# xiaochuanle/MECAT

Measured on AMD Instinct MI355X. Metric: candidate overlaps/sec, higher is better.
Workload: dtype int32

## Files before the change

### mecat_amd/csrc/seed_strand.hip

```cpp
#include <stdlib.h>

#include <algorithm>

#include "seed_defs.h"
#include "seed_replay.h"
#include "seed_walk.h"

#define FS_CAP 8192
#define FS_SEGCAP 6144
#define FS_SMALLN 16
#define FS_BIGN 512
#define FS_BIGCAP 768
#define FS_GATECAP 1024
#define FS_OVF16 0x8000u
#ifndef FS_Q1
#define FS_LPB1 8
#define FS_NP1 4
#define FS_Q1 2
#define FS_D1 2
#define FS_LPB2 8
#define FS_NP2 4
#define FS_Q2 2
#define FS_D2 2
#endif

struct FsLds {
    union {
        uint32_t cnt32[FLT_M / 2];
        struct {
            uint32_t pay[FS_CAP];
            uint16_t eslot[FS_CAP];
            uint16_t big[FS_BIGCAP];
            uint32_t hist[FS_WAVES][64];
            uint64_t tf[FS_GATECAP];
        } e;
    } x;
    union {
        uint32_t cur32[FS_CAP / 2];
        uint16_t perm[FS_SEGCAP];
    } y;
    uint32_t occ[REL_WORDS];
    uint32_t rel[REL_WORDS];
    uint16_t base_ci[REL_WORDS];
    uint32_t sq_id[FS_SEGCAP];
    uint16_t sq_st[FS_SEGCAP + 2];
    uint16_t sq_score[FS_SEGCAP];
    uint16_t gate[FS_GATECAP];
    uint32_t qpos[FS_WAVES][128];
    uint16_t qkm[FS_WAVES][128];
    uint32_t wtot[FS_WAVES];
    unsigned long long red[FS_WAVES];
    unsigned long long tally[3];
    uint32_t misc[12];
};
static_assert(sizeof(FsLds) <= 160 * 1024 - 512, "one workgroup per CU");

struct FusedCtl { unsigned long long alloc; unsigned int n_fallback; unsigned int next ; unsigned long long prof[32]; };
#ifdef FS_PROF
#define FS_MARK(i) do { __syncthreads(); if (threadIdx.x == 0) { const unsigned long long t_ = wall_clock64(); atomicAdd(&ctl->prof[(i) + 16 * (s & 1)], t_ - t_prev); t_prev = t_; } } while (0)
#else
#define FS_MARK(i) do { } while (0)
#endif

__device__ __forceinline__ void fs_block_sum2(const int tid, uint32_t a, uint32_t b, unsigned long long* red , uint32_t* sa, uint32_t* sb) {
    const int lane = tid & 63;
    for (int o = 32; o > 0; o >>= 1) {
        a += (uint32_t)__builtin_amdgcn_ds_bpermute((lane ^ o) << 2, (int)a);
        b += (uint32_t)__builtin_amdgcn_ds_bpermute((lane ^ o) << 2, (int)b);
    }
    const unsigned long long v = (unsigned long long)a | ((unsigned long long)b << 32);
    if (lane == 0) red[tid >> 6] = v;
    __syncthreads();
    unsigned long long t = 0;
#pragma unroll
    for (int w = 0; w < FS_WAVES; ++w) t += red[w];
    *sa = (uint32_t)t;
    *sb = (uint32_t)(t >> 32);
}

struct FsStrand { int rid, off, len, K, cut_byte; bool rev; };
__device__ __forceinline__ FsStrand fs_strand(const mhip_offset_t* __restrict__ roffs, const ReadSel& sel, int ib, int s, bool cuts, int cut_step) {
    FsStrand d;
    d.rid = sel_rid(sel, ib + (s >> 1));
    d.off = roffs[d.rid].offset;
    d.len = roffs[d.rid].size;
    d.K = kmers_of(d.len);
    d.rev = s & 1;
    d.cut_byte = 7;
    if (cuts) {
        const long long need = (long long)d.off + d.len + 1 + 5 * ZV;
        const long long t = (need + cut_step - 1) / cut_step;
        if (t <= 7) d.cut_byte = (int)t - 1;
    }
    return d;
}
__device__ __forceinline__ int64_t fs_kmer_at(const FsStrand& d, int km) {
    return !d.rev ? (int64_t)d.off + (int64_t)km * BC : (int64_t)d.off + d.len - MHIP_KMER_SIZE - (int64_t)km * BC;
}
__device__ __forceinline__ void fs_hdr_words(const uint32_t* __restrict__ pac, const FsStrand& d, int km, uint32_t (&w)[2]) {
    const int64_t i = fs_kmer_at(d, km) >> 4;
    w[0] = pac[i];
    w[1] = pac[i + 1];
}
__device__ __forceinline__ void fs_hdr_record(const uint32_t* __restrict__ starts, const uint4* __restrict__ recs, const FsStrand& d, int km,
                                              const uint32_t (&w)[2], uint32_t (&r)[3]) {
    const uint64_t W = ((uint64_t)__builtin_bswap32(w[0]) << 32) | __builtin_bswap32(w[1]);
    uint32_t id = (uint32_t)(W >> (64 - 26 - (int)((fs_kmer_at(d, km) & 15) << 1))) & KMER_MASK;
    if (d.rev) id = kmer_revcomp(id);
    if (recs) {
        const uint4 v = recs[id];
        r[0] = v.x; r[1] = v.y; r[2] = v.z;
    } else {
        r[0] = starts[id]; r[1] = starts[id + 1];
    }
}
__device__ __forceinline__ void fs_hdr_decode(bool cuts, const FsStrand& d, const uint32_t (&r)[3], uint32_t* bs, uint32_t* cnt, uint32_t* all) {
    *bs = r[0];
    if (cuts) {
        *all = r[2] >> 24;
        *cnt = ((d.cut_byte < 4 ? r[1] : r[2]) >> (8 * (d.cut_byte & 3))) & 0xFFu;
    } else {
        *all = *cnt = r[1] - r[0];
    }
}

template <int NQ>
__device__ __forceinline__ void fs_bitonic(uint32_t* p, const uint32_t n, const int lane) {
    uint32_t v[NQ];
#pragma unroll
    for (int q = 0; q < NQ; ++q) { const uint32_t idx = q * 64 + lane; v[q] = idx < n ? p[idx] : 0xFFFFFFFFu; }
#pragma unroll
    for (int k = 2; k <= NQ * 64; k <<= 1) {
#pragma unroll
        for (int j = k >> 1; j > 0; j >>= 1) {
            if (j >= 64) {
                const int dq = j >> 6;
#pragma unroll
                for (int q = 0; q < NQ; ++q) {
                    if ((q & dq) == 0) {
                        const uint32_t a = v[q], b = v[q | dq];
                        const bool asc = ((q * 64) & k) == 0;
                        v[q] = asc ? min(a, b) : max(a, b);
                        v[q | dq] = asc ? max(a, b) : min(a, b);
                    }
                }
            } else {
#pragma unroll
                for (int q = 0; q < NQ; ++q) {
                    const uint32_t o = (uint32_t)__builtin_amdgcn_ds_bpermute((lane ^ j) << 2, (int)v[q]);
                    const bool asc = (((q * 64 + lane) & k) == 0), lower = (lane & j) == 0;
                    v[q] = (asc == lower) ? min(v[q], o) : max(v[q], o);
                }
            }
        }
    }
    __builtin_amdgcn_wave_barrier();
#pragma unroll
    for (int q = 0; q < NQ; ++q) { const uint32_t idx = q * 64 + lane; if (idx < n) p[idx] = v[q]; }
}

__device__ __forceinline__ uint32_t fs_cnt(const uint32_t* cnt32, uint32_t e) { return (cnt32[e >> 1] >> ((e & 1u) * 16u)) & 0xFFFFu; }

#define FS_UNI(x) ((uint32_t)__builtin_amdgcn_readfirstlane((int)(x)))
__global__ __launch_bounds__(FS_THREADS) void seed_strand(const uint32_t* __restrict__ pac, const mhip_offset_t* __restrict__ roffs, ReadSel sel,
                                                          int ib, int ns, const uint32_t* __restrict__ starts, const uint4* __restrict__ recs,
                                                          int cut_step, const uint16_t* __restrict__ slots, const int32_t* __restrict__ offsets,
                                                          SeedArrays A, int gate, int hi_bits, int min_kmer_match, double cutoff,
                                                          unsigned long long cap, FusedCtl* __restrict__ ctl,
                                                          unsigned long long* __restrict__ counters, RefReads R) {
    __shared__ FsLds L;
    const int tid0 = threadIdx.x;
    const bool probed = A.km_bstart != nullptr;
    const bool cuts = recs != nullptr;
    uint32_t* const hbs = L.sq_id;
    uint16_t* const hcn = L.sq_score;
    constexpr int PF = 2;
    uint32_t pw[PF][2], pr[PF][3];
#pragma unroll
    for (int j = 0; j < PF; ++j) { pw[j][0] = pw[j][1] = 0; pr[j][0] = pr[j][1] = pr[j][2] = 0; }
    int pf = -1;
    if (tid0 == 0) { L.tally[0] = L.tally[1] = L.tally[2] = 0; L.misc[8] = atomicAdd(&ctl->next, 1u); L.misc[9] = atomicAdd(&ctl->next, 1u); }
    __syncthreads();
    int s = (int)min(FS_UNI(L.misc[8]), (uint32_t)ns), sn = (int)min(FS_UNI(L.misc[9]), (uint32_t)ns), s2 = ns;
    for (; s < ns; s = sn, sn = s2) {
    __syncthreads();
    int tid = tid0;
    asm volatile("" : "+v"(tid));
    const int lane = tid & 63, wv = __builtin_amdgcn_readfirstlane(tid >> 6);
    const FsStrand d = fs_strand(roffs, sel, ib, s, cuts, cut_step);
    const int rid = d.rid, rlen = d.len, K = d.K;
    auto fail = [&]() {
        if (tid == 0) { A.fused[s] = 0; atomicAdd(&ctl->n_fallback, 1u); atomicAdd(&counters[14], 1ull); }
    };
    unsigned long long t_prev = wall_clock64(); (void)t_prev;
    for (int i = tid; i < FLT_M / 2; i += FS_THREADS) L.x.cnt32[i] = 0;
    for (int i = tid; i < REL_WORDS; i += FS_THREADS) L.rel[i] = 0u;
    if (tid < 8) L.misc[tid] = 0;
    if (tid == 0) L.misc[8] = atomicAdd(&ctl->next, 1u);
    uint32_t Hall, run_all;
    {
        const bool room = K <= FS_SEGCAP;
        uint32_t hc = 0, ha = 0;
        if (probed) {
            const uint32_t kb = A.km_base[s];
            for (int km = tid; km < K; km += FS_THREADS) {
                const uint32_t bs = A.km_bstart[kb + km], cn = A.km_cnt[kb + km];
                hc += cn;
                if (room) { hbs[km] = bs; hcn[km] = (uint16_t)cn; }
            }
        } else {
            auto take = [&](int km, const uint32_t (&r)[3]) {
                uint32_t bs, cn, al;
                fs_hdr_decode(cuts, d, r, &bs, &cn, &al);
                hc += cn;
                ha += al;
                if (room) { hbs[km] = bs; hcn[km] = (uint16_t)cn; }
            };
            if (pf != s) {
#pragma unroll
                for (int j = 0; j < PF; ++j)
                    if (tid + j * FS_THREADS < K) fs_hdr_words(pac, d, tid + j * FS_THREADS, pw[j]);
#pragma unroll
                for (int j = 0; j < PF; ++j)
                    if (tid + j * FS_THREADS < K) fs_hdr_record(starts, recs, d, tid + j * FS_THREADS, pw[j], pr[j]);
            }
#pragma unroll
            for (int j = 0; j < PF; ++j) asm volatile("" : "+v"(pr[j][0]), "+v"(pr[j][1]), "+v"(pr[j][2]));
#pragma unroll
            for (int j = 0; j < PF; ++j)
                if (tid + j * FS_THREADS < K) take(tid + j * FS_THREADS, pr[j]);
            for (int km = tid + PF * FS_THREADS; km < K; km += FS_THREADS) {
                uint32_t w[2], r[3] = {0, 0, 0};
                fs_hdr_words(pac, d, km, w);
                fs_hdr_record(starts, recs, d, km, w, r);
                take(km, r);
            }
        }
        fs_block_sum2(tid, hc, ha, L.red, &Hall, &run_all);
        Hall = FS_UNI(Hall);
        run_all = FS_UNI(run_all);
        s2 = (int)min(FS_UNI(L.misc[8]), (uint32_t)ns);
        if (!probed && tid == 0) { L.tally[0] += (unsigned long long)K; L.tally[1] += run_all; L.tally[2] += Hall; A.strand_hits_all[s] = Hall; }
    }
    if (Hall == 0) {
        if (tid == 0) { A.fused[s] = 1; A.strand_hits[s] = 0; A.hit_base[s] = 0; A.nseg[s] = 0; A.nrec[s] = 0; A.ngated[s] = 0; }
        continue;
    }
    if (Hall >= 65536u || K > 32767 || K > FS_SEGCAP) { fail(); continue; }

    FS_MARK(0);
    fs_walk<FS_LPB1, FS_NP1, FS_Q1, FS_D1, false>(tid, hbs, hcn, slots, K, [&](int, uint32_t e) { atomicAdd(&L.x.cnt32[e >> 1], 1u << ((e & 1u) * 16u)); });
    __syncthreads();
    FS_MARK(1);

    static_assert(FLT_M / FS_THREADS == 32, "one bitmap word per thread");
    uint32_t cw[18];
    {
        const uint4* c4 = (const uint4*)&L.x.cnt32[16 * tid];
#pragma unroll
        for (int q = 0; q < 4; ++q) { const uint4 v = c4[q]; cw[1 + 4 * q] = v.x; cw[2 + 4 * q] = v.y; cw[3 + 4 * q] = v.z; cw[4 + 4 * q] = v.w; }
        cw[0] = L.x.cnt32[(16 * tid - 1) & (FLT_M / 2 - 1)];
        cw[17] = L.x.cnt32[(16 * tid + 16) & (FLT_M / 2 - 1)];
        uint32_t hot = 0;
        {
#pragma unroll
        for (int j = 1; j <= 16; ++j) {
            const int lo = (int)(cw[j] & 0xFFFFu), hi = (int)(cw[j] >> 16), pl = (int)(cw[j - 1] >> 16), nx = (int)(cw[j + 1] & 0xFFFFu);
            const bool hl = lo > 0 && (lo + hi >= gate || lo + pl >= gate);
            const bool hh = hi > 0 && (hi + nx >= gate || hi + lo >= gate);
            hot |= (hl ? 1u : 0u) << (2 * (j - 1)) | (hh ? 1u : 0u) << (2 * (j - 1) + 1);
        }
        const uint32_t reach = (uint32_t)min(sweep_reach(rlen), FLT_M / 2 - 1);
        for (uint32_t m = hot; m; m &= m - 1u) {
            const uint32_t e = (uint32_t)tid * 32u + (uint32_t)__builtin_ctz(m);
            uint32_t lo = (e - reach) & (FLT_M - 1), left = 2 * reach + 1;
            while (left > 0) {
                const uint32_t b = lo & 31u, take = min(32u - b, left);
                const uint32_t msk = (take == 32u ? 0xFFFFFFFFu : ((1u << take) - 1u)) << b;
                atomicOr(&L.rel[lo >> 5], msk);
                lo = (lo + take) & (FLT_M - 1);
                left -= take;
            }
        }
        }
    }
    __syncthreads();
    FS_MARK(2);
    uint32_t kept;
    {
        const uint32_t r = L.rel[tid];
        uint32_t occ = 0, mine = 0;
        bool toolong = false;
#pragma unroll
        for (int j = 0; j < 32; ++j) {
            const uint32_t h = (cw[1 + (j >> 1)] >> ((j & 1) * 16)) & 0xFFFFu;
            if (((r >> j) & 1u) && h) { occ |= 1u << j; mine += h; toolong |= h > FS_BIGN; }
        }
        uint32_t both;
        const uint32_t exb = fs_excl_scan(tid, mine | ((uint32_t)__popc(occ) << 16), L.wtot, &both);
        const uint32_t ex = exb & 0xFFFFu, cx = exb >> 16;
        kept = FS_UNI(both) & 0xFFFFu;
        if (kept > FS_CAP) { fail(); continue; }
        L.occ[tid] = occ;
        L.base_ci[tid] = (uint16_t)cx;
        uint16_t* cur16 = (uint16_t*)L.y.cur32;
        uint32_t at = ex, ci = cx;
        if (occ) {
#pragma unroll
            for (int j = 0; j < 32; ++j) {
                const uint32_t h = (cw[1 + (j >> 1)] >> ((j & 1) * 16)) & 0xFFFFu;
                if ((occ >> j) & 1u) { cur16[ci++] = (uint16_t)at; at += h; }
            }
        }
        if (toolong) L.misc[3] = 1;
        __syncthreads();
        if (FS_UNI(L.misc[3])) { fail(); continue; }
    }
    if (kept == 0) {
        if (tid == 0) { A.fused[s] = 1; A.strand_hits[s] = 0; A.hit_base[s] = 0; A.nseg[s] = 0; A.nrec[s] = 0; A.ngated[s] = 0; }
        continue;
    }
    if (tid == 0) {
        const unsigned long long hb0 = atomicAdd(&ctl->alloc, (unsigned long long)kept);
        if (hb0 + kept > cap) L.misc[3] = 1;
        L.misc[6] = (uint32_t)hb0;
        L.misc[7] = (uint32_t)(hb0 >> 32);
    }
    __syncthreads();
    if (FS_UNI(L.misc[3])) { fail(); continue; }
    const uint64_t hb = ((uint64_t)L.misc[7] << 32) | L.misc[6];

    FS_MARK(3);
    const bool ahead = !probed && sn < ns;
    FsStrand dn = d;
    if (ahead) {
        dn = fs_strand(roffs, sel, ib, sn, cuts, cut_step);
#pragma unroll
        for (int j = 0; j < PF; ++j)
            if (tid + j * FS_THREADS < dn.K) fs_hdr_words(pac, dn, tid + j * FS_THREADS, pw[j]);
    }
    {
        uint32_t qn = 0;
        auto place = [&](uint32_t qi) {
            const uint32_t pos = L.qpos[wv][qi], km = L.qkm[wv][qi];
            const uint32_t seg = pos / (uint32_t)ZV, off = pos - seg * (uint32_t)ZV;
            const uint32_t e = seg & (FLT_M - 1), w = e >> 5, b = e & 31u;
            const uint32_t oc = L.occ[w];
            const uint32_t ci = (uint32_t)L.base_ci[w] + (uint32_t)__popc(oc & ((1u << b) - 1u));
            const uint32_t sh = (ci & 1u) * 16u;
            const uint32_t p = (atomicAdd(&L.y.cur32[ci >> 1], 1u << sh) >> sh) & 0xFFFFu;
            L.x.e.pay[p] = ((seg >> FLT_BITS) << 26) | (km << 11) | off;
            L.x.e.eslot[p] = (uint16_t)e;
        };
        fs_walk<FS_LPB2, FS_NP2, FS_Q2, FS_D2, true>(tid, hbs, hcn, offsets, K, [&](int km, uint32_t pos, bool valid) {
            const uint32_t seg = pos / (uint32_t)ZV;
            const uint32_t e = seg & (FLT_M - 1);
            const uint32_t oc = valid ? L.occ[e >> 5] : 0u;
            const bool keep = (bool)((oc >> (e & 31u)) & 1u);
            const unsigned long long m = __builtin_amdgcn_ballot_w64(keep);
            if (m) {
                if (keep) {
                    const uint32_t at = qn + (uint32_t)__popcll(m & ((1ull << lane) - 1ull));
                    L.qpos[wv][at] = pos;
                    L.qkm[wv][at] = (uint16_t)km;
                }
                qn += (uint32_t)__popcll(m);
                if (qn >= 64u) { qn -= 64u; place(qn + (uint32_t)lane); }
            }
        });
        if ((uint32_t)lane < qn) place((uint32_t)lane);
    }
    if (ahead) {
#pragma unroll
        for (int j = 0; j < PF; ++j)
            if (tid + j * FS_THREADS < dn.K) fs_hdr_record(starts, recs, dn, tid + j * FS_THREADS, pw[j], pr[j]);
        pf = sn;
    }
    __syncthreads();
    FS_MARK(4);
    {
        const uint16_t* cur16 = (const uint16_t*)L.y.cur32;
        uint32_t val[FS_CAP / FS_THREADS], dst[FS_CAP / FS_THREADS];
#pragma unroll
        for (int rd = 0; rd < FS_CAP / FS_THREADS; ++rd) {
            const uint32_t i = (uint32_t)rd * FS_THREADS + tid;
            dst[rd] = 0xFFFFFFFFu;
            val[rd] = 0;
            if ((uint32_t)rd * FS_THREADS < kept && i < kept) {
                const uint32_t v = L.x.e.pay[i], e = L.x.e.eslot[i], w = e >> 5, oc = L.occ[w];
                const uint32_t ci = (uint32_t)L.base_ci[w] + (uint32_t)__popc(oc & ((1u << (e & 31u)) - 1u));
                const uint32_t st = ci ? cur16[ci - 1] : 0u, en = cur16[ci], n = en - st;
                if (n > FS_SMALLN) {
                    if (i == st) L.x.e.big[atomicAdd(&L.misc[0], 1u)] = (uint16_t)ci;
                } else if (n > 1) {
                    uint32_t rank = 0;
                    for (uint32_t k = st; k < en; ++k) rank += L.x.e.pay[k] < v ? 1u : 0u;
                    val[rd] = v;
                    dst[rd] = st + rank;
                }
            }
        }
        __syncthreads();
#pragma unroll
        for (int rd = 0; rd < FS_CAP / FS_THREADS; ++rd)
            if (dst[rd] != 0xFFFFFFFFu) L.x.e.pay[dst[rd]] = val[rd];
        FS_MARK(11);
        const uint32_t nbig = L.misc[0];
        for (uint32_t k = wv; k < nbig; k += FS_WAVES) {
            const uint32_t ci = L.x.e.big[k];
            const uint32_t st = ci ? cur16[ci - 1] : 0u, n = (uint32_t)cur16[ci] - st;
            if (n <= 64) fs_bitonic<1>(L.x.e.pay + st, n, lane);
            else if (n <= 256) fs_bitonic<4>(L.x.e.pay + st, n, lane);
            else fs_bitonic<8>(L.x.e.pay + st, n, lane);
        }
        __syncthreads();
    }

    FS_MARK(5);
    uint32_t nrec, nseg;
    {
        constexpr int CHMAX = FS_CAP / FS_THREADS;
        const uint32_t ch = (kept + FS_THREADS - 1) / FS_THREADS;
        const uint32_t i0 = (uint32_t)tid * ch;
        uint32_t pv[CHMAX], sv[CHMAX];
        uint32_t ppay = 0, psl = 0xFFFFFFFFu;
        if (i0 > 0 && i0 < kept) { ppay = L.x.e.pay[i0 - 1]; psl = L.x.e.eslot[i0 - 1]; }
        uint32_t hm = 0, rm = 0;
#pragma unroll
        for (int c = 0; c < CHMAX; ++c) {
            const uint32_t i = i0 + c;
            const bool in = (uint32_t)c < ch && i < kept;
            pv[c] = in ? L.x.e.pay[i] : 0u;
            sv[c] = in ? L.x.e.eslot[i] : 0u;
            const bool head = in && (sv[c] != psl || (pv[c] >> 26) != (ppay >> 26));
            const bool rec = in && (head || ((pv[c] >> 11) & 0x7FFFu) != ((ppay >> 11) & 0x7FFFu));
            hm |= (head ? 1u : 0u) << c;
            rm |= (rec ? 1u : 0u) << c;
            if (in) { ppay = pv[c]; psl = sv[c]; }
        }
        uint32_t both;
        const uint32_t ex = fs_excl_scan(tid, (uint32_t)__popc(rm) | ((uint32_t)__popc(hm) << 16), L.wtot, &both);
        uint32_t rpos = ex & 0xFFFFu, spos = ex >> 16;
        both = FS_UNI(both);
        nrec = both & 0xFFFFu;
        nseg = both >> 16;
        if (nseg > FS_SEGCAP) { fail(); continue; }
#pragma unroll
        for (int c = 0; c < CHMAX; ++c) {
            if ((rm >> c) & 1u) {
                if ((hm >> c) & 1u) {
                    L.sq_id[spos] = ((pv[c] >> 26) << FLT_BITS) | sv[c];
                    L.sq_st[spos] = (uint16_t)rpos;
                    ++spos;
                }
                L.x.e.pay[rpos++] = ((pv[c] & 0x7FFu) << 16) | ((((pv[c] >> 11) & 0x7FFFu) + 1u) & 0xFFFFu);
            }
        }
        if (tid == 0) L.sq_st[nseg] = (uint16_t)nrec;
    }
    uint16_t* perm = L.y.perm;
    __syncthreads();

    FS_MARK(6);
    if (hi_bits == 0) {
        for (uint32_t q = tid; q < nseg; q += FS_THREADS) perm[q] = (uint16_t)q;
    } else {
        uint32_t* hist = &L.x.e.hist[0][0];
        hist[tid] = 0;
        __syncthreads();
        const uint32_t chunk = (((nseg + FS_WAVES - 1) / FS_WAVES) + 63u) & ~63u;
        const uint32_t lo = min(nseg, (uint32_t)wv * chunk), hi = min(nseg, lo + chunk);
        for (uint32_t q = lo + lane; q < hi; q += 64) atomicAdd(&L.x.e.hist[wv][L.sq_id[q] >> FLT_BITS], 1u);
        __syncthreads();
        {
            const uint32_t bin = tid >> 4, w = tid & 15;
            static_assert(FS_WAVES == 16, "16 waves");
            const uint32_t v = L.x.e.hist[w][bin];
            uint32_t all;
            const uint32_t ex = fs_excl_scan(tid, v, L.wtot, &all);
            L.x.e.hist[w][bin] = ex;
        }
        __syncthreads();
        volatile uint32_t* cur = L.x.e.hist[wv];
        const uint64_t lt = (1ull << lane) - 1ull;
        for (uint32_t q0 = lo; q0 < hi; q0 += 64) {
            const uint32_t q = q0 + lane;
            const bool valid = q < hi;
            const uint32_t d = valid ? L.sq_id[q] >> FLT_BITS : 0u;
            uint64_t peers = __ballot(valid);
            for (int b = 0; b < hi_bits; ++b) {
                const uint64_t m = __ballot((d >> b) & 1u);
                peers &= ((d >> b) & 1u) ? m : ~m;
            }
            const uint32_t rank = __popcll(peers & lt);
            const uint32_t base = valid ? cur[d] : 0u;
            if (valid) perm[base + rank] = (uint16_t)q;
            if (valid && rank == 0) cur[d] = base + (uint32_t)__popcll(peers);
        }
    }
    FS_MARK(7);
    uint16_t* ovf = L.x.e.big;
    for (uint32_t q = tid; q < nseg; q += FS_THREADS) {
        const uint32_t c = (uint32_t)L.sq_st[q + 1] - (uint32_t)L.sq_st[q];
        if (c > SM) {
            const uint32_t k = atomicAdd(&L.misc[1], 1u);
            if (k < FS_BIGCAP) ovf[k] = (uint16_t)q;
            L.sq_score[q] = (uint16_t)FS_OVF16;
        } else {
            L.sq_score[q] = (uint16_t)c;
        }
    }
    __syncthreads();
    if (FS_UNI(L.misc[1]) > FS_BIGCAP) { fail(); continue; }
    {
        const uint32_t novf = L.misc[1];
        for (uint32_t k = wv; k < novf; k += FS_WAVES) {
            const uint32_t q = ovf[k];
            const uint32_t st = L.sq_st[q], en = L.sq_st[q + 1];
            int sc;
            replay_overflow(L.x.e.pay + st, (int)(en - st), A.ent_fin + hb + st, A.escore + hb + st, cutoff, &sc);
            if (lane == 0) L.sq_score[q] = (uint16_t)((uint32_t)sc | FS_OVF16);
        }
    }
    __syncthreads();
    FS_MARK(8);
    for (uint32_t g = tid; g < nseg; g += FS_THREADS) {
        const uint32_t q = perm[g];
        const uint32_t sid = L.sq_id[q];
        int s_k = (int)(L.sq_score[q] & 0x7FFFu);
        if (g > 0 && sid > 0) {
            const uint32_t ql = perm[g - 1];
            if (L.sq_id[ql] == sid - 1u) {
                const uint32_t st = L.sq_st[ql], en = L.sq_st[ql + 1];
                const uint32_t t = L.x.e.pay[(uint32_t)L.sq_st[q + 1] - 1u] & 0xFFFFu;
                uint32_t lo = st, hi = en;
                while (lo < hi) {
                    const uint32_t mid = (lo + hi) >> 1;
                    if ((L.x.e.pay[mid] & 0xFFFFu) <= t) lo = mid + 1; else hi = mid;
                }
                if (lo > st) s_k += (L.sq_score[ql] & FS_OVF16) ? (int)A.escore[hb + lo - 1] : (int)(lo - st);
            }
        }
        bool listed = (int)(int16_t)s_k >= 2 * min_kmer_match;
        if (listed && R.enable) listed = !subjects_all_higher(R, sid, rid, roffs[rid].offset + rlen + 1);
        if (listed) {
            const uint32_t k = atomicAdd(&L.misc[2], 1u);
            if (k < FS_GATECAP) {
                const uint32_t e0 = L.x.e.pay[L.sq_st[q]];
                L.gate[k] = (uint16_t)g;
                L.x.e.tf[k] = ((uint64_t)((e0 & 0xFFFFu) - 1u) << 32) | (uint64_t)(sid * (uint32_t)ZV + (e0 >> 16));
            }
        }
    }
    __syncthreads();
    const uint32_t ng = FS_UNI(L.misc[2]);
    if (ng > FS_GATECAP) { fail(); continue; }
    FS_MARK(9);
    for (uint32_t a = tid; a < ng; a += FS_THREADS) {
        const uint64_t ta = L.x.e.tf[a];
        uint32_t rank = 0;
        for (uint32_t b = 0; b < ng; ++b) rank += L.x.e.tf[b] < ta ? 1u : 0u;
        A.gated[hb + rank] = (uint32_t)L.gate[a];
    }
    for (uint32_t i = tid; i < nrec; i += FS_THREADS) A.ent[hb + i] = L.x.e.pay[i];
    for (uint32_t g = tid; g < nseg; g += FS_THREADS) {
        const uint32_t q = perm[g];
        const uint32_t sc = L.sq_score[q];
        A.seg_id[hb + g] = L.sq_id[q];
        A.seg_start[hb + g] = L.sq_st[q];
        A.seg_score[hb + g] = (int32_t)((sc & 0x7FFFu) | ((sc & FS_OVF16) ? OVF_FLAG : 0u));
    }
    FS_MARK(10);
    if (tid == 0) {
        atomicAdd(&counters[13], 1ull);
        A.fused[s] = 1;
        A.strand_hits[s] = kept;
        A.hit_base[s] = hb;
        A.nseg[s] = nseg;
        A.nrec[s] = nrec;
        A.ngated[s] = ng;
    }
    }
    if (!probed && tid0 == 0) {
        atomicAdd(&counters[0], L.tally[0]);
        atomicAdd(&counters[1], L.tally[1]);
        if (cuts) atomicAdd(&counters[15], L.tally[2]);
    }
}

#undef FS_UNI

static int print_strand_stats(const SeedBatch& b) {
    const int ns = b.ns;
    std::vector<uint32_t> h[5];
    const uint32_t* src[5] = {b.A.strand_hits_all, b.F.strand_hits, b.F.nseg, b.F.nrec, b.F.ngated};
    for (int i = 0; i < 5; ++i) { h[i].resize((size_t)ns); HIPCHK(hipMemcpy(h[i].data(), src[i], sizeof(uint32_t) * (size_t)ns, hipMemcpyDeviceToHost)); }
    std::vector<int32_t> fu((size_t)ns);
    HIPCHK(hipMemcpy(fu.data(), b.A.fused, sizeof(int32_t) * (size_t)ns, hipMemcpyDeviceToHost));
    for (int s = 0; s < ns; ++s)
        if (fu[(size_t)s]) fprintf(stderr, "SEEDSTAT %d %u %u %u %u %u\n", s & 1, h[0][(size_t)s], h[1][(size_t)s], h[2][(size_t)s], h[3][(size_t)s], h[4][(size_t)s]);
    return 0;
}

int seed_run_strand(SeedBatch& b, unsigned int* n_fallback) {
    mhip_ctx* c = b.c;
    SeedArrays& F = b.F;
    const int ns = b.ns;
    size_t capF = (size_t)((double)b.sumK * b.hits_per_lookup / 5.0) + (size_t)ns * 256 + 64;
    if (b.knobs.fused_room > 0) capF = (size_t)b.knobs.fused_room;
    FusedCtl* d_ctl;
    if (c->scratch("sf_ctl", sizeof(FusedCtl), (void**)&d_ctl)) return -1;
    if (seed_strand_tables(c, "sf_", ns, &F)) return -1;
    if (seed_hit_tables(c, "sf_", capF, &F)) return -1;
    HIPCHK(hipMemsetAsync(d_ctl, 0, sizeof(FusedCtl), c->stream));
    LAUNCH(c, "seed_strand", seed_strand, std::min(ns, std::max(1, c->num_cus)), FS_THREADS, 0, (const uint32_t*)b.reads->d_pac,
           (const mhip_offset_t*)b.reads->d_offs, b.sel, b.ib, ns, (const uint32_t*)b.idx->d_starts, b.recs, b.cut_step,
           (const uint16_t*)b.idx->d_slots, (const int32_t*)b.idx->d_offsets, F, b.gate, std::max(0, b.nbits - FLT_BITS), (int)b.P->min_kmer_match,
           b.P->ddfs_cutoff, (unsigned long long)capF, d_ctl, (unsigned long long*)c->d_counters, b.RR);
    FusedCtl ctl;
    HIPCHK(hipMemcpyAsync(&ctl, d_ctl, sizeof(ctl), hipMemcpyDeviceToHost, c->stream));
    HIPCHK(hipStreamSynchronize(c->stream));
    *n_fallback = ctl.n_fallback;
#ifdef FS_PROF
    for (int i = 0; i < 12; ++i) fprintf(stderr, "FS_PROF phase %d: F %.1f R %.1f us per strand\n", i, (double)ctl.prof[i] / 50.0 / ns, (double)ctl.prof[i + 16] / 50.0 / ns);
#endif
    if (getenv("MECAT_SEED_STATS")) return print_strand_stats(b);
    return 0;
}
```

### mecat_amd/csrc/seed_walk.h

```cpp
#pragma once

#include "seed_defs.h"

#define FS_THREADS 1024
#define FS_WAVES (FS_THREADS / WAVE)

__device__ __forceinline__ uint32_t fs_excl_scan(const int tid, uint32_t v, uint32_t* wtot, uint32_t* total) {
    const int lane = tid & 63, wave = tid >> 6;
    uint32_t incl = v;
    for (int o = 1; o < 64; o <<= 1) {
        const uint32_t n = (uint32_t)__builtin_amdgcn_ds_bpermute(((lane - o) & 63) << 2, (int)incl);
        if (lane >= o) incl += n;
    }
    __syncthreads();
    if (lane == 63) wtot[wave] = incl;
    __syncthreads();
    uint32_t base = 0, tot = 0;
#pragma unroll
    for (int w = 0; w < FS_WAVES; ++w) {
        const uint32_t x = wtot[w];
        if (w < wave) base += x;
        tot += x;
    }
    *total = tot;
    return base + incl - v;
}

template <int LPB, int NP, int Q, int D, bool UNIFORM, typename T, typename C, typename F>
__device__ __forceinline__ void fs_walk(const int tid, const uint32_t* __restrict__ kbs, const C* __restrict__ kcn, const T* __restrict__ arr,
                                        const int K, F f) {
    constexpr int G = FS_THREADS / LPB, STEP = Q * G;
    const int g = tid / LPB;
    const uint32_t sub = (uint32_t)tid % LPB;
    uint32_t hb[Q], hc[Q];
    uint32_t sb[D][Q], sc[D][Q], sd[D][Q][NP];
#define FS_HDR(BASE, BS, CN)                                                      \
    _Pragma("unroll") for (int q = 0; q < Q; ++q) {                               \
        const int km_ = (BASE) + q * G + g;                                       \
        BS[q] = km_ < K ? kbs[km_] : 0u;                                          \
        CN[q] = km_ < K ? (uint32_t)kcn[km_] : 0u;                                \
    }
#define FS_DAT(BS, CN, DD)                                                        \
    _Pragma("unroll") for (int q = 0; q < Q; ++q)                                 \
        _Pragma("unroll") for (int p = 0; p < NP; ++p)                            \
            DD[q][p] = sub + (uint32_t)(p * LPB) < CN[q] ? (uint32_t)arr[BS[q] + (uint32_t)(p * LPB) + sub] : 0u;
#pragma unroll
    for (int d = 0; d < D; ++d) { FS_HDR(d * STEP, sb[d], sc[d]) }
    FS_HDR(D * STEP, hb, hc)
#pragma unroll
    for (int d = 0; d < D; ++d) { FS_DAT(sb[d], sc[d], sd[d]) }
    for (int base = 0; base < K; base += STEP) {
        uint32_t cb[Q], cc[Q], cd[Q][NP];
#pragma unroll
        for (int q = 0; q < Q; ++q) {
            cb[q] = sb[0][q]; cc[q] = sc[0][q];
#pragma unroll
            for (int p = 0; p < NP; ++p) cd[q][p] = sd[0][q][p];
        }
#pragma unroll
        for (int d = 0; d + 1 < D; ++d)
#pragma unroll
            for (int q = 0; q < Q; ++q) {
                sb[d][q] = sb[d + 1][q]; sc[d][q] = sc[d + 1][q];
#pragma unroll
                for (int p = 0; p < NP; ++p) sd[d][q][p] = sd[d + 1][q][p];
            }
#pragma unroll
        for (int q = 0; q < Q; ++q) { sb[D - 1][q] = hb[q]; sc[D - 1][q] = hc[q]; }
        FS_DAT(sb[D - 1], sc[D - 1], sd[D - 1])
        FS_HDR(base + (D + 1) * STEP, hb, hc)
#pragma unroll
        for (int q = 0; q < Q; ++q) {
            const int km = base + q * G + g;
            if constexpr (UNIFORM) {
#pragma unroll
                for (int p = 0; p < NP; ++p) {
                    const bool v = sub + (uint32_t)(p * LPB) < cc[q];
                    if (__any(v)) f(km, cd[q][p], v);
                }
                for (uint32_t r = (uint32_t)(NP * LPB) + sub; __any(r < cc[q]); r += 4 * LPB) {
                    uint32_t tv[4];
#pragma unroll
                    for (int u = 0; u < 4; ++u) tv[u] = r + (uint32_t)(u * LPB) < cc[q] ? (uint32_t)arr[cb[q] + r + (uint32_t)(u * LPB)] : 0u;
#pragma unroll
                    for (int u = 0; u < 4; ++u) { const bool v = r + (uint32_t)(u * LPB) < cc[q]; if (__any(v)) f(km, tv[u], v); }
                }
            } else {
#pragma unroll
                for (int p = 0; p < NP; ++p)
                    if (sub + (uint32_t)(p * LPB) < cc[q]) f(km, cd[q][p]);
                for (uint32_t r = (uint32_t)(NP * LPB) + sub; r < cc[q]; r += 4 * LPB) {
                    uint32_t tv[4];
#pragma unroll
                    for (int u = 0; u < 4; ++u) tv[u] = r + (uint32_t)(u * LPB) < cc[q] ? (uint32_t)arr[cb[q] + r + (uint32_t)(u * LPB)] : 0u;
#pragma unroll
                    for (int u = 0; u < 4; ++u) if (r + (uint32_t)(u * LPB) < cc[q]) f(km, tv[u]);
                }
            }
        }
    }
#undef FS_HDR
#undef FS_DAT
}
```

Measured before the change: 7.305 million.

## Pack bucket gating into 16-bit SIMD ops and batch walk-2 occ lookups

The per-bucket hot and occupancy tests now use packed 16-bit vector arithmetic on the two counts in each word, with bit interleave and split helpers mapping between packed and natural bit order. The per-bucket prefix loop becomes a walk over set bits that reads counts from LDS. The second walk callback now receives all four pieces of a bucket at once and issues their occ loads together, ballot-compacting with mbcnt to overlap LDS latency. The aim is fewer scalar ALU ops and better latency hiding, at the cost of more register pressure, more LDS reads in the set-bit loop, and some asm barriers.

```diff
diff --git a/mecat_amd/csrc/seed_strand.hip b/mecat_amd/csrc/seed_strand.hip
--- a/mecat_amd/csrc/seed_strand.hip
+++ b/mecat_amd/csrc/seed_strand.hip
@@ -23,6 +23,10 @@
 #define FS_Q2 2
 #define FS_D2 2
 #endif
+#ifndef FS_W2B
+#define FS_W2B 2
+#endif
+static_assert(FS_NP2 == 4 && (FS_W2B == 2 || FS_W2B == 4), "walk 2 takes a bucket's four pieces in halves or together");
 
 struct FsLds {
     union {
@@ -161,6 +165,19 @@
 
 __device__ __forceinline__ uint32_t fs_cnt(const uint32_t* cnt32, uint32_t e) { return (cnt32[e >> 1] >> ((e & 1u) * 16u)) & 0xFFFFu; }
 
+typedef unsigned short fs_u16x2 __attribute__((ext_vector_type(2)));
+__device__ __forceinline__ fs_u16x2 fs_pk(uint32_t x) { return __builtin_bit_cast(fs_u16x2, x); }
+__device__ __forceinline__ uint32_t fs_unpk(fs_u16x2 x) { return __builtin_bit_cast(uint32_t, x); }
+__device__ __forceinline__ uint32_t fs_swap_step(uint32_t x, int s, uint32_t m) { const uint32_t t = (x ^ (x >> s)) & m; return x ^ t ^ (t << s); }
+__device__ __forceinline__ uint32_t fs_interleave(uint32_t x) {
+    x = fs_swap_step(x, 8, 0x0000FF00u); x = fs_swap_step(x, 4, 0x00F000F0u); x = fs_swap_step(x, 2, 0x0C0C0C0Cu);
+    return fs_swap_step(x, 1, 0x22222222u);
+}
+__device__ __forceinline__ uint32_t fs_split(uint32_t x) {
+    x = fs_swap_step(x, 1, 0x22222222u); x = fs_swap_step(x, 2, 0x0C0C0C0Cu); x = fs_swap_step(x, 4, 0x00F000F0u);
+    return fs_swap_step(x, 8, 0x0000FF00u);
+}
+
 #define FS_UNI(x) ((uint32_t)__builtin_amdgcn_readfirstlane((int)(x)))
 __global__ __launch_bounds__(FS_THREADS) void seed_strand(const uint32_t* __restrict__ pac, const mhip_offset_t* __restrict__ roffs, ReadSel sel,
                                                           int ib, int ns, const uint32_t* __restrict__ starts, const uint4* __restrict__ recs,
@@ -255,24 +272,32 @@
 
     static_assert(FLT_M / FS_THREADS == 32, "one bitmap word per thread");
     uint32_t cw[18];
+    uint32_t nes = 0;
     {
         const uint4* c4 = (const uint4*)&L.x.cnt32[16 * tid];
 #pragma unroll
         for (int q = 0; q < 4; ++q) { const uint4 v = c4[q]; cw[1 + 4 * q] = v.x; cw[2 + 4 * q] = v.y; cw[3 + 4 * q] = v.z; cw[4 + 4 * q] = v.w; }
         cw[0] = L.x.cnt32[(16 * tid - 1) & (FLT_M / 2 - 1)];
         cw[17] = L.x.cnt32[(16 * tid + 16) & (FLT_M / 2 - 1)];
-        uint32_t hot = 0;
         {
+        const uint16_t g1 = (uint16_t)min(max(gate - 1, 0), 65535);
+        uint32_t one32 = 0x00010001u;
+        asm volatile("" : "+s"(one32));
+        const fs_u16x2 gm1 = {g1, g1}, one = fs_pk(one32);
+        uint32_t hs = 0;
 #pragma unroll
         for (int j = 1; j <= 16; ++j) {
-            const int lo = (int)(cw[j] & 0xFFFFu), hi = (int)(cw[j] >> 16), pl = (int)(cw[j - 1] >> 16), nx = (int)(cw[j + 1] & 0xFFFFu);
-            const bool hl = lo > 0 && (lo + hi >= gate || lo + pl >= gate);
-            const bool hh = hi > 0 && (hi + nx >= gate || hi + lo >= gate);
-            hot |= (hl ? 1u : 0u) << (2 * (j - 1)) | (hh ? 1u : 0u) << (2 * (j - 1) + 1);
+            const fs_u16x2 c = fs_pk(cw[j]);
+            const fs_u16x2 lf = fs_pk(__builtin_amdgcn_alignbit(cw[j], cw[j - 1], 16)), rt = fs_pk(__builtin_amdgcn_alignbit(cw[j + 1], cw[j], 16));
+            const fs_u16x2 sum = c + __builtin_elementwise_max(lf, rt);
+            const fs_u16x2 t = __builtin_elementwise_min(__builtin_elementwise_sub_sat(sum, gm1), c);
+            hs |= fs_unpk(__builtin_elementwise_min(t, one)) << (j - 1);
+            nes |= fs_unpk(__builtin_elementwise_min(c, one)) << (j - 1);
         }
         const uint32_t reach = (uint32_t)min(sweep_reach(rlen), FLT_M / 2 - 1);
-        for (uint32_t m = hot; m; m &= m - 1u) {
-            const uint32_t e = (uint32_t)tid * 32u + (uint32_t)__builtin_ctz(m);
+        for (uint32_t m = hs; m; m &= m - 1u) {
+            const uint32_t k = (uint32_t)__builtin_ctz(m);
+            const uint32_t e = (uint32_t)tid * 32u + (((k & 15u) << 1) | (k >> 4));
             uint32_t lo = (e - reach) & (FLT_M - 1), left = 2 * reach + 1;
             while (left > 0) {
                 const uint32_t b = lo & 31u, take = min(32u - b, left);
@@ -288,14 +313,17 @@
     FS_MARK(2);
     uint32_t kept;
     {
-        const uint32_t r = L.rel[tid];
-        uint32_t occ = 0, mine = 0;
-        bool toolong = false;
-#pragma unroll
-        for (int j = 0; j < 32; ++j) {
-            const uint32_t h = (cw[1 + (j >> 1)] >> ((j & 1) * 16)) & 0xFFFFu;
-            if (((r >> j) & 1u) && h) { occ |= 1u << j; mine += h; toolong |= h > FS_BIGN; }
-        }
+        const uint32_t od = fs_split(L.rel[tid]) & nes;
+        const uint32_t occ = fs_interleave(od);
+        fs_u16x2 hsum = {0, 0}, hmax = {0, 0};
+#pragma unroll
+        for (int j = 1; j <= 16; ++j) {
+            const fs_u16x2 h = fs_pk(cw[j]) * fs_pk((od >> (j - 1)) & 0x00010001u);
+            hsum += h;
+            hmax = __builtin_elementwise_max(hmax, h);
+        }
+        const uint32_t mine = (uint32_t)hsum.x + (uint32_t)hsum.y;
+        const bool toolong = max((uint32_t)hmax.x, (uint32_t)hmax.y) > FS_BIGN;
         uint32_t both;
         const uint32_t exb = fs_excl_scan(tid, mine | ((uint32_t)__popc(occ) << 16), L.wtot, &both);
         const uint32_t ex = exb & 0xFFFFu, cx = exb >> 16;
@@ -305,12 +333,9 @@
         L.base_ci[tid] = (uint16_t)cx;
         uint16_t* cur16 = (uint16_t*)L.y.cur32;
         uint32_t at = ex, ci = cx;
-        if (occ) {
-#pragma unroll
-            for (int j = 0; j < 32; ++j) {
-                const uint32_t h = (cw[1 + (j >> 1)] >> ((j & 1) * 16)) & 0xFFFFu;
-                if ((occ >> j) & 1u) { cur16[ci++] = (uint16_t)at; at += h; }
-            }
+        for (uint32_t m = occ; m; m &= m - 1u) {
+            cur16[ci++] = (uint16_t)at;
+            at += fs_cnt(L.x.cnt32, (uint32_t)tid * 32u + (uint32_t)__builtin_ctz(m));
         }
         if (toolong) L.misc[3] = 1;
         __syncthreads();
@@ -352,20 +377,30 @@
             L.x.e.pay[p] = ((seg >> FLT_BITS) << 26) | (km << 11) | off;
             L.x.e.eslot[p] = (uint16_t)e;
         };
-        fs_walk<FS_LPB2, FS_NP2, FS_Q2, FS_D2, true>(tid, hbs, hcn, offsets, K, [&](int km, uint32_t pos, bool valid) {
-            const uint32_t seg = pos / (uint32_t)ZV;
-            const uint32_t e = seg & (FLT_M - 1);
-            const uint32_t oc = valid ? L.occ[e >> 5] : 0u;
-            const bool keep = (bool)((oc >> (e & 31u)) & 1u);
-            const unsigned long long m = __builtin_amdgcn_ballot_w64(keep);
-            if (m) {
-                if (keep) {
-                    const uint32_t at = qn + (uint32_t)__popcll(m & ((1ull << lane) - 1ull));
-                    L.qpos[wv][at] = pos;
-                    L.qkm[wv][at] = (uint16_t)km;
+        fs_walk<FS_LPB2, FS_NP2, FS_Q2, FS_D2, true>(tid, hbs, hcn, offsets, K, [&](int km, const uint32_t (&pos)[4], const bool (&valid)[4]) {
+#pragma unroll
+            for (int h = 0; h < 4; h += FS_W2B) {
+                uint32_t e[FS_W2B], oc[FS_W2B];
+#pragma unroll
+                for (int p = 0; p < FS_W2B; ++p) e[p] = (pos[h + p] / (uint32_t)ZV) & (FLT_M - 1);
+#pragma unroll
+                for (int p = 0; p < FS_W2B; ++p) oc[p] = L.occ[e[p] >> 5];
+#pragma unroll
+                for (int p = 0; p < FS_W2B; ++p) {
+                    uint32_t kb = ((valid[h + p] ? oc[p] : 0u) >> (e[p] & 31u)) & 1u;
+                    asm volatile("" : "+v"(kb));
+                    const bool keep = kb != 0u;
+                    const unsigned long long m = __builtin_amdgcn_ballot_w64(keep);
+                    if (m) {
+                        if (keep) {
+                            const uint32_t at = __builtin_amdgcn_mbcnt_hi((uint32_t)(m >> 32), __builtin_amdgcn_mbcnt_lo((uint32_t)m, qn));
+                            L.qpos[wv][at] = pos[h + p];
+                            L.qkm[wv][at] = (uint16_t)km;
+                        }
+                        qn += (uint32_t)__popcll(m);
+                        if (qn >= 64u) { qn -= 64u; place(qn + (uint32_t)lane); }
+                    }
                 }
-                qn += (uint32_t)__popcll(m);
-                if (qn >= 64u) { qn -= 64u; place(qn + (uint32_t)lane); }
             }
         });
         if ((uint32_t)lane < qn) place((uint32_t)lane);
@@ -518,7 +553,9 @@
             const uint32_t q = ovf[k];
             const uint32_t st = L.sq_st[q], en = L.sq_st[q + 1];
             int sc;
-            replay_overflow(L.x.e.pay + st, (int)(en - st), A.ent_fin + hb + st, A.escore + hb + st, cutoff, &sc);
+            uint32_t* fin = A.ent_fin + hb + st;
+            asm volatile("" : "+v"(fin));
+            replay_overflow(L.x.e.pay + st, (int)(en - st), fin, A.escore + hb + st, cutoff, &sc);
             if (lane == 0) L.sq_score[q] = (uint16_t)((uint32_t)sc | FS_OVF16);
         }
     }
diff --git a/mecat_amd/csrc/seed_walk.h b/mecat_amd/csrc/seed_walk.h
--- a/mecat_amd/csrc/seed_walk.h
+++ b/mecat_amd/csrc/seed_walk.h
@@ -73,17 +73,19 @@
         for (int q = 0; q < Q; ++q) {
             const int km = base + q * G + g;
             if constexpr (UNIFORM) {
+                bool v[NP];
 #pragma unroll
-                for (int p = 0; p < NP; ++p) {
-                    const bool v = sub + (uint32_t)(p * LPB) < cc[q];
-                    if (__any(v)) f(km, cd[q][p], v);
-                }
+                for (int p = 0; p < NP; ++p) v[p] = sub + (uint32_t)(p * LPB) < cc[q];
+                if (__any(v[0])) f(km, cd[q], v);
                 for (uint32_t r = (uint32_t)(NP * LPB) + sub; __any(r < cc[q]); r += 4 * LPB) {
                     uint32_t tv[4];
+                    bool tok[4];
 #pragma unroll
-                    for (int u = 0; u < 4; ++u) tv[u] = r + (uint32_t)(u * LPB) < cc[q] ? (uint32_t)arr[cb[q] + r + (uint32_t)(u * LPB)] : 0u;
-#pragma unroll
-                    for (int u = 0; u < 4; ++u) { const bool v = r + (uint32_t)(u * LPB) < cc[q]; if (__any(v)) f(km, tv[u], v); }
+                    for (int u = 0; u < 4; ++u) {
+                        tok[u] = r + (uint32_t)(u * LPB) < cc[q];
+                        tv[u] = tok[u] ? (uint32_t)arr[cb[q] + r + (uint32_t)(u * LPB)] : 0u;
+                    }
+                    f(km, tv, tok);
                 }
             } else {
 #pragma unroll
```

Result: no change. 7.338 million (median of 6 runs) (+0.5%).
